# 0xMiden/miden-vm

Hardware: AMD Instinct MI355X
Metric: trace rows/sec proved (2^20-row trace, 96-bit sec) (higher is better)
Workload: dtype u64 (Goldilocks field, p = 2^64 - 2^32 + 1); 1 GPU; full proof of miden:20:51:8 (DummyMidenAir 2^20 x 51 + 8 EF aux), 96-bit production PCS params (blowup 8, FRI arity 4, 27 queries, PoW 4/12/16), Poseidon2 LMCS; trace resident in HBM, transcript on host; log_trace_rows=20, main_width=51, aux_width_ef=8, log_blowup=3, proof_bytes=137697, parallelism=1 GPU

## Files before the change

### miden-vm_amd/csrc/fri.hip

```cpp
#include <cstring>
#include "gl.cuh"
#include "../../include/midenhip.h"
#include "kernels.hpp"
#include "blake3.cuh"
#include "keccak.cuh"
#include "poseidon2_fast.cuh"
#define RESCUE_FAST 1
#include "rescue.cuh"
#include "salt.cuh"

__device__ __forceinline__ e2 ld_e2(const u64* p, size_t idx) {
  const ulonglong2 v = *reinterpret_cast<const ulonglong2*>(p + 2 * idx);
  return e2{v.x, v.y};
}
__device__ __forceinline__ void st_e2(u64* p, size_t idx, e2 v) { *reinterpret_cast<ulonglong2*>(p + 2 * idx) = make_ulonglong2(v.c0, v.c1); }

__device__ __forceinline__ u32 fri_row_pos(u32 p, int log_arity) { return bitrev32(p, log_arity); }

template <bool SALT>
__device__ __forceinline__ void fri_leaf_hash_body(const u64* __restrict__ ev, int log_rows , int cbits, int log_arity,
                                                   u64* __restrict__ digests, const SaltArgs* sa) {
  const int log_q = log_rows - log_arity;
  const size_t leaves = (size_t)1 << (log_q + cbits);
  const size_t s = blockIdx.x * (size_t)256 + threadIdx.x;
  if (s >= leaves) return;
  const size_t j = s >> log_q, r0 = s & (((size_t)1 << log_q) - 1);
  const u32 arity = 1u << log_arity;
  u64 st[12];
#pragma unroll
  for (int i = 0; i < 12; i++) st[i] = 0;
  for (u32 p0 = 0; p0 < arity; p0 += 4) {
#pragma unroll
    for (u32 k = 0; k < 4; k++) {
      e2 v = e2_make(0);
      if (p0 + k < arity) v = ld_e2(ev, (j << log_rows) + r0 + ((size_t)fri_row_pos(p0 + k, log_arity) << log_q));
      st[2 * k] = (p0 + k < arity) ? v.c0 : 0;
      st[2 * k + 1] = (p0 + k < arity) ? v.c1 : 0;
    }
    p2f_permute(st);
  }
  if constexpr (SALT) salt_absorb_p2(st, *sa, salt_phys_row(j, r0, cbits, log_q + cbits));
  ulonglong2* o = reinterpret_cast<ulonglong2*>(digests + 4 * s);
  o[0] = make_ulonglong2(st[0], st[1]);
  o[1] = make_ulonglong2(st[2], st[3]);
}
__global__ __launch_bounds__(256) void k_fri_leaf_hash(const u64* __restrict__ ev, int log_rows, int cbits, int log_arity,
                                                       u64* __restrict__ digests) {
  fri_leaf_hash_body<false>(ev, log_rows, cbits, log_arity, digests, nullptr);
}
__global__ __launch_bounds__(256) void k_fri_leaf_hash_salted(const u64* __restrict__ ev, int log_rows, int cbits, int log_arity,
                                                              u64* __restrict__ digests, SaltArgs sa) {
  fri_leaf_hash_body<true>(ev, log_rows, cbits, log_arity, digests, &sa);
}

template <bool SALT>
__device__ __forceinline__ void fri_leaf_hash_b3_body(const u64* __restrict__ ev, int log_rows, int cbits, int log_arity,
                                                      u64* __restrict__ digests, const SaltArgs* sa) {
  const int log_q = log_rows - log_arity;
  const size_t leaves = (size_t)1 << (log_q + cbits);
  const size_t s = blockIdx.x * (size_t)256 + threadIdx.x;
  if (s >= leaves) return;
  const size_t j = s >> log_q, r0 = s & (((size_t)1 << log_q) - 1);
  const u32 arity = 1u << log_arity;
  const u32 total = 32 + 16 * arity, n_blocks = (total + 63) / 64;
  b3::Stream h;
  h.init();
  uint32_t m[16], out[8];
#pragma unroll 1
  for (u32 b = 0; b < n_blocks; b++) {
    const int p0 = (int)(4 * b) - 2;
#pragma unroll
    for (int k = 0; k < 4; k++) {
      const int pp = p0 + k;
      e2 v = e2_make(0);
      if (pp >= 0 && (u32)pp < arity) v = ld_e2(ev, (j << log_rows) + r0 + ((size_t)fri_row_pos((u32)pp, log_arity) << log_q));
      m[4 * k] = (uint32_t)v.c0; m[4 * k + 1] = (uint32_t)(v.c0 >> 32);
      m[4 * k + 2] = (uint32_t)v.c1; m[4 * k + 3] = (uint32_t)(v.c1 >> 32);
    }
    if (b + 1 < n_blocks) h.block(m);
    else h.finish(m, total - 64 * b, out);
  }
  if constexpr (SALT) salt_absorb_b3(out, *sa, salt_phys_row(j, r0, cbits, log_q + cbits));
#pragma unroll
  for (int i = 0; i < 4; i++) digests[4 * s + i] = (u64)out[2 * i] | ((u64)out[2 * i + 1] << 32);
}
__global__ __launch_bounds__(256) void k_fri_leaf_hash_b3(const u64* __restrict__ ev, int log_rows, int cbits, int log_arity,
                                                          u64* __restrict__ digests) {
  fri_leaf_hash_b3_body<false>(ev, log_rows, cbits, log_arity, digests, nullptr);
}
__global__ __launch_bounds__(256) void k_fri_leaf_hash_b3_salted(const u64* __restrict__ ev, int log_rows, int cbits, int log_arity,
                                                                 u64* __restrict__ digests, SaltArgs sa) {
  fri_leaf_hash_b3_body<true>(ev, log_rows, cbits, log_arity, digests, &sa);
// ... 387 lines not shown
```

### miden-vm_amd/csrc/lmcs.hip

```cpp
#include "ctx.hpp"
#include "../../include/midenhip.h"
#include "kernels.hpp"
#include "poseidon2_fast.cuh"
#include "poseidon2_lanes.cuh"
#include "poseidon2_quad.cuh"
#include "blake3.cuh"
#include "keccak.cuh"
#define RESCUE_FAST 1
#include "rescue.cuh"
#include "gl.cuh"
#include "salt.cuh"
#include <algorithm>
#include <cstring>

static constexpr int LEAF_MAX_MATS = 8;
static constexpr int LEAF_THREADS = 256;

__global__ __launch_bounds__(256) void k_permute_soa(u64* st, size_t n) {
  size_t i = blockIdx.x * (size_t)blockDim.x + threadIdx.x;
  if (i >= n) return;
  u64 s[12];
#pragma unroll
  for (int j = 0; j < 12; j++) s[j] = st[j * n + i];
  p2f_permute(s);
// ... 20 lines not shown
double poseidon2_register_rate(mh_ctx* c) {
  const int blocks = 2048, iters = 64;
  DevBuf out((size_t)blocks * 256 * 8);
  hipEvent_t a = c->get_event(), b = c->get_event();
  MH_LAUNCH(k_perm_rate, dim3(blocks), dim3(256), 0, c->stream, out.u(), iters, 1ULL);
  double best = 0;
  for (int rep = 0; rep < 3; rep++) {
    HIP_CHECK(hipEventRecord(a, c->stream));
    MH_LAUNCH(k_perm_rate, dim3(blocks), dim3(256), 0, c->stream, out.u(), iters, 12345ULL + rep);
    HIP_CHECK(hipEventRecord(b, c->stream));
    HIP_CHECK(hipStreamSynchronize(c->stream));
    float ms = 0;
    HIP_CHECK(hipEventElapsedTime(&ms, a, b));
    best = std::max(best, (double)blocks * 256 * iters / (ms * 1e-3));
  }
  c->event_pool.push_back(a);
  c->event_pool.push_back(b);
  return best;
}

struct LeafMat {
  const u64* data;
  u32 width;
};
struct LeafArgs {
  LeafMat m[LEAF_MAX_MATS];
  int n_mats;
  int log_blowup;
  int log_n;
  const u64* state_in;
  int log_n_prev;
  u64* state_out;
  u64* digest_out;
  size_t q_begin, q_count;
};

template <bool SALT>
__device__ __forceinline__ void leaf_absorb_body(const LeafArgs& a, const SaltArgs* sa) {
  const size_t leaves = (size_t)1 << (a.log_n + a.log_blowup);
  const size_t q = a.q_begin + blockIdx.x * (size_t)blockDim.x + threadIdx.x;
  if (q >= (a.q_count ? a.q_begin + a.q_count : leaves)) return;
  const size_t j = q >> a.log_n, r = q & (((size_t)1 << a.log_n) - 1);
  u64 s[12];
  if (a.state_in) {
    const size_t leaves_prev = (size_t)1 << (a.log_n_prev + a.log_blowup);
    const size_t qi = (j << a.log_n_prev) + (r & (((size_t)1 << a.log_n_prev) - 1));
#pragma unroll
    for (int i = 0; i < 12; i++) s[i] = a.state_in[i * leaves_prev + qi];
  } else {
#pragma unroll
    for (int i = 0; i < 12; i++) s[i] = 0;
  }
  const size_t col_stride = leaves;
#pragma unroll 1
  for (int mi = 0; mi < a.n_mats; mi++) {
    const u64* base = a.m[mi].data + q;
    const u32 w = a.m[mi].width;
#pragma unroll 1
    for (u32 c0 = 0; c0 < w; c0 += 8) {
#pragma unroll
      for (int k = 0; k < 8; k++) s[k] = (c0 + k < w) ? base[(size_t)(c0 + k) * col_stride] : 0;
      p2f_permute(s);
    }
  }
  if constexpr (SALT) salt_absorb_p2(s, *sa, salt_phys_row(j, r, a.log_blowup, a.log_n + a.log_blowup));
  if (a.digest_out) {
    ulonglong2* o = reinterpret_cast<ulonglong2*>(a.digest_out + 4 * q);
    o[0] = make_ulonglong2(s[0], s[1]);
    o[1] = make_ulonglong2(s[2], s[3]);
  } else {
#pragma unroll
    for (int i = 0; i < 12; i++) a.state_out[i * leaves + q] = s[i];
  }
}
__global__ __launch_bounds__(LEAF_THREADS) void k_leaf_absorb(LeafArgs a) { leaf_absorb_body<false>(a, nullptr); }
__global__ __launch_bounds__(LEAF_THREADS) void k_leaf_absorb_salted(LeafArgs a, SaltArgs sa) { leaf_absorb_body<true>(a, &sa); }

template <bool SALT>
__device__ __forceinline__ void leaf_absorb_b3_body(const LeafArgs& a, const SaltArgs* sa) {
  const size_t leaves = (size_t)1 << (a.log_n + a.log_blowup);
  const size_t q = a.q_begin + blockIdx.x * (size_t)blockDim.x + threadIdx.x;
  if (q >= (a.q_count ? a.q_begin + a.q_count : leaves)) return;
  const size_t j = q >> a.log_n, r = q & (((size_t)1 << a.log_n) - 1);
  uint32_t st[8];
  if (a.state_in) {
    const size_t qi = (j << a.log_n_prev) + (r & (((size_t)1 << a.log_n_prev) - 1));
#pragma unroll
    for (int i = 0; i < 4; i++) {
      const u64 v = a.state_in[4 * qi + i];
      st[2 * i] = (uint32_t)v;
      st[2 * i + 1] = (uint32_t)(v >> 32);
    }
  } else {
#pragma unroll
    for (int i = 0; i < 8; i++) st[i] = 0;
  }
  const size_t col_stride = leaves;
#pragma unroll 1
  for (int mi = 0; mi < a.n_mats; mi++) {
    const u64* base = a.m[mi].data + q;
    const u32 w = a.m[mi].width;
    const u32 total = 32 + 8 * w;
    const u32 n_blocks = (total + 63) / 64;
    b3::Stream h;
    h.init();
    uint32_t m[16];
#pragma unroll 1
    for (u32 b = 0; b < n_blocks; b++) {
      const int f0 = (int)(8 * b) - 4;
#pragma unroll
      for (int k = 0; k < 8; k++) {
        const int f = f0 + k;
        u64 v = 0;
        if (f >= 0 && (u32)f < w) v = base[(size_t)f * col_stride];
        m[2 * k] = (uint32_t)v;
// ... 180 lines not shown
    if (e < sa.n) out[k * (size_t)sa.n + e] = z[e];
}
void lmcs_salt_rows(mh_ctx* c, const SaltArgs& salt, const u64* rows, size_t n_rows, u64* out) {
  if (!n_rows || !salt.n) return;
  MH_LAUNCH(k_salt_rows, dim3((unsigned)((n_rows + 255) / 256)), dim3(256), 0, c->stream, salt, rows, n_rows, out);
}
void lmcs_salt_assign(mh_ctx* c, mh_tree* t) {
  if (!c->salt.n) return;
  t->salt = c->salt;
  c->salt.tree++;
}
const SaltArgs* lmcs_salt_of(const mh_tree* t) { return t->salt.n ? &t->salt : nullptr; }
__global__ __launch_bounds__(256) void k_compress_kk(const u64* __restrict__ in, u64* __restrict__ out, size_t n_out, int log_n_coset) {
  const size_t q = blockIdx.x * (size_t)256 + threadIdx.x;
  if (q >= n_out) return;
  size_t l, rgt;
  if (log_n_coset >= 0) {
    const size_t N = (size_t)1 << log_n_coset;
    const size_t jp = q >> log_n_coset, r = q & (N - 1);
    l = ((2 * jp) << log_n_coset) + r;
    rgt = l + N;
  } else {
    l = 2 * q;
    rgt = l + 1;
  }
  uint64_t a[4], b[4], o[4];
#pragma unroll
  for (int i = 0; i < 4; i++) {
    a[i] = in[4 * l + i];
    b[i] = in[4 * rgt + i];
  }
  kk::compress_pair(a, b, o);
#pragma unroll
  for (int i = 0; i < 4; i++) out[4 * q + i] = o[i];
}

__global__ __launch_bounds__(256) void k_compress(const u64* __restrict__ in, u64* __restrict__ out, size_t n_out, int log_n_coset) {
  const size_t q = blockIdx.x * (size_t)blockDim.x + threadIdx.x;
  if (q >= n_out) return;
  size_t l, rgt;
  if (log_n_coset >= 0) {
    size_t N = (size_t)1 << log_n_coset;
    size_t jp = q >> log_n_coset, r = q & (N - 1);
    l = ((2 * jp) << log_n_coset) + r;
    rgt = l + N;
  } else {
    l = 2 * q;
    rgt = l + 1;
  }
  const ulonglong2* pl = reinterpret_cast<const ulonglong2*>(in + 4 * l);
  const ulonglong2* pr = reinterpret_cast<const ulonglong2*>(in + 4 * rgt);
  ulonglong2 l0 = pl[0], l1 = pl[1], r0 = pr[0], r1 = pr[1];
  u64 s[12] = {l0.x, l0.y, l1.x, l1.y, r0.x, r0.y, r1.x, r1.y, 0, 0, 0, 0};
  p2f_permute(s);
  ulonglong2* o = reinterpret_cast<ulonglong2*>(out + 4 * q);
  o[0] = make_ulonglong2(s[0], s[1]);
  o[1] = make_ulonglong2(s[2], s[3]);
}

static size_t compress_lanes_max_nodes() {
  static const size_t v = [] {
    const char* e = getenv("MH_LANES_MAX_NODES");
    return e ? (size_t)atol(e) : (size_t)8192;
  }();
  return v;
}
__global__ __launch_bounds__(256) void k_compress_lanes(const u64* __restrict__ in, u64* __restrict__ out, size_t n_out, int log_n_coset) {
  const size_t node = (blockIdx.x * (size_t)256 + threadIdx.x) >> 4;
  const int g = threadIdx.x & 15;
  const bool active = node < n_out;
  const size_t q = active ? node : 0;
  size_t l, rgt;
  if (log_n_coset >= 0) {
    const size_t N = (size_t)1 << log_n_coset;
    const size_t jp = q >> log_n_coset, r = q & (N - 1);
    l = ((2 * jp) << log_n_coset) + r;
    rgt = l + N;
  } else {
    l = 2 * q;
    rgt = l + 1;
  }
  const u64* src = in + 4 * (g < 4 ? l : rgt) + (g & 3);
  u64 s = g < 8 ? *src : 0;
  s = p2l_permute(s);
  if (active && g < 4) out[4 * q + g] = s;
}

static size_t compress_quad_min_nodes() {
  static const size_t v = [] {
    const char* e = getenv("MH_QUAD_MIN_NODES");
    return e ? (size_t)atol(e) : (size_t)16384;
  }();
  return v;
}
static size_t compress_quad_max_nodes() {
  static const size_t v = [] {
    const char* e = getenv("MH_QUAD_MAX_NODES");
    return e ? (size_t)atol(e) : (size_t)32768;
  }();
  return v;
}
__global__ __launch_bounds__(256) void k_compress_quad(const u64* __restrict__ in, u64* __restrict__ out, size_t n_out, int log_n_coset) {
  const size_t node = (blockIdx.x * (size_t)256 + threadIdx.x) >> 2;
  const int j = threadIdx.x & 3;
  const bool active = node < n_out;
  const size_t q = active ? node : 0;
  size_t l, rgt;
// ... 388 lines not shown
```

### miden-vm_amd/csrc/p2_fast_constants.inc

```
static const unsigned long long P2F_ARK_INT_SCALED[22] = {
  0x4adf842aa75d4316ULL, 0xc7ddc3945255a751ULL, 0x3a16dbc6b75abaa6ULL, 0x4160d6694e06fff1ULL,
  0xe022996682de326cULL, 0xc8e9d874293bba12ULL, 0xa2e2b15ade3b7d8fULL, 0x9b6dac180ec943cfULL,
  0xe8bb7136f94d695dULL, 0xf12458f8ebe4789bULL, 0x1dc193fff01be2b6ULL, 0xb68e807d90fed489ULL,
  0x1e4085d70c946015ULL, 0x66a5e58521b4c3c6ULL, 0x53b280ba8b2f8249ULL, 0xe4d602af8c2cf37eULL,
  0x813ee2a294c44327ULL, 0x813b943e27068773ULL, 0x9abe7bd4fb69436eULL, 0x12f583e142599766ULL,
  0x3798883e37881f6bULL, 0xed264b0c16fc039fULL,
};
static const unsigned long long P2F_INT_K[22] = {
  0x0000000000000001ULL, 0xffffbfff00004001ULL, 0xefffffff00000001ULL, 0xfffffbff00000001ULL,
  0xfffffffeff000001ULL, 0xfffffffeffffffc1ULL, 0x000ffffffff00000ULL, 0x00000003fffffffcULL,
  0x0001000000000000ULL, 0x0000000040000000ULL, 0x0000000000001000ULL, 0xfbffffff04000001ULL,
  0xfffffeff00000101ULL, 0xffbfffff00000001ULL, 0xffffffef00000001ULL, 0xfffffffefffc0001ULL,
  0xffffffff00000000ULL, 0x00003fffffffc000ULL, 0x1000000000000000ULL, 0x0000040000000000ULL,
  0x0000000001000000ULL, 0x0000000000000040ULL,
};
static const unsigned long long P2F_DESCALE = 0xfffffffec0000001ULL;
static const unsigned long long P2G_ARK[22] = {
  0x4adf842aa75d4316ULL, 0x8fbb8729a4ab4ea1ULL, 0x742db78d6eb5754cULL, 0x82c1acd29c0dffe2ULL,
  0xc04532ce05bc64d7ULL, 0x91d3b0e952777423ULL, 0x45c562b6bc76fb1dULL, 0x36db58311d92879dULL,
  0xd176e26ef29ad2b9ULL, 0xe248b1f2d7c8f135ULL, 0x3b8327ffe037c56cULL, 0x6d1d00fc21fda911ULL,
  0x3c810bae1928c02aULL, 0xcd4bcb0a4369878cULL, 0xa7650175165f0492ULL, 0xc9ac05601859e6fbULL,
  0x027dc5462988864dULL, 0x0277287d4e0d0ee5ULL, 0x357cf7aaf6d286dbULL, 0x25eb07c284b32eccULL,
  0x6f31107c6f103ed6ULL, 0xda4c96192df8073dULL,
};
static const unsigned long long P2G_K[22] = {
  0x0000000000000002ULL, 0xfffffeff00000101ULL, 0xffbfffff00000001ULL, 0xffffffef00000001ULL,
  0xfffffffefffc0001ULL, 0xffffffff00000000ULL, 0x00003fffffffc000ULL, 0x1000000000000000ULL,
  0x0000040000000000ULL, 0x0000000001000000ULL, 0x0000000000000040ULL, 0xffefffff00100001ULL,
  0xfffffffb00000005ULL, 0xfffeffff00000001ULL, 0xfffffffec0000001ULL, 0xfffffffefffff001ULL,
  0x03fffffffc000000ULL, 0x000000ffffffff00ULL, 0x0040000000000000ULL, 0x0000001000000000ULL,
  0x0000000000040000ULL, 0x0000000000000001ULL,
};
static const unsigned long long P2G_DESCALE = 0xfffffffee0000001ULL;
static constexpr int P2F_INT_K_LOG2[22] = {0, 174, 156, 138, 120, 102, 84, 66, 48, 30, 12, 186, 168, 150, 132, 114, 96, 78, 60, 42, 24, 6};
static constexpr int P2F_DESCALE_LOG2 = 126;
static constexpr int P2G_K_LOG2[22] = {1, 168, 150, 132, 114, 96, 78, 60, 42, 24, 6, 180, 162, 144, 126, 108, 90, 72, 54, 36, 18, 0};
static constexpr int P2G_DESCALE_LOG2 = 125;
```

### miden-vm_amd/csrc/poseidon2_fast.cuh

```cuda
#pragma once
#include "poseidon2.cuh"

namespace p2c {
#include "p2_fast_constants.inc"
}

#ifndef P2F_ASM
#define P2F_ASM 1
#endif
#ifndef P2F_GROUP
#define P2F_GROUP 4
#endif

#if defined(__HIP_DEVICE_COMPILE__)

template <u32 K>
__device__ __forceinline__ u64 p2f_mad(u64 acc, u32 x) {
  u64 d, cy;
  asm("v_mad_u64_u32 %0, %1, %2, %3, %4" : "=v"(d), "=s"(cy) : "v"(x), "n"(K), "v"(acc));
  return d;
}
template <u32 K>
__device__ __forceinline__ u64 p2f_zmul(u32 x) {
  u64 d, cy;
  asm("v_mad_u64_u32 %0, %1, %2, %3, 0" : "=v"(d), "=s"(cy) : "v"(x), "n"(K));
  return d;
}
__device__ __forceinline__ u32 lo32(u64 x) { return (u32)x; }
__device__ __forceinline__ u32 hi32(u64 x) { return (u32)(x >> 32); }

__device__ __forceinline__ u64 p2f_mul_c(u64 a, u64 b) {
  const u32 a0 = lo32(a), a1 = hi32(a), b0 = lo32(b), b1 = hi32(b);
  const u64 p00 = (u64)a0 * b0;
  const u64 m = (u64)a0 * b1 + (p00 >> 32);
  const u64 m2 = (u64)a1 * b0 + (u32)m;
  const u64 hi = (u64)a1 * b1 + (m >> 32) + (m2 >> 32);
  const u64 lo = (m2 << 32) | (u32)p00;
  const u32 x2 = lo32(hi), x3 = hi32(hi);
  u64 t = (u64)x2 * 0xFFFFFFFFu + lo;
  t += (t < lo) ? GL_EPS : 0;
  u64 r = t - x3;
  r -= (t < x3) ? GL_EPS : 0;
  return r;
}
#define P2F_A asm volatile
#ifndef P2F_GAP_NOPS
#define P2F_GAP_NOPS 1
#endif
#define P2F_GAP()                                          \
  do {                                                     \
    if (P2F_GAP_NOPS && N == 1) P2F_A("s_nop 1");          \
    else if (P2F_GAP_NOPS && N == 2) P2F_A("s_nop 0");     \
  } while (0)
#define P2F_SCR(i, PRE, POST, ...)                                                  \
  do {                                                                              \
    switch ((i) & 7) {                                                              \
      case 0: P2F_A(PRE "s[84:85]" POST : __VA_ARGS__ : "s84", "s85"); break;        \
      case 1: P2F_A(PRE "s[86:87]" POST : __VA_ARGS__ : "s86", "s87"); break;        \
      case 2: P2F_A(PRE "s[88:89]" POST : __VA_ARGS__ : "s88", "s89"); break;        \
      case 3: P2F_A(PRE "s[90:91]" POST : __VA_ARGS__ : "s90", "s91"); break;        \
      case 4: P2F_A(PRE "s[92:93]" POST : __VA_ARGS__ : "s92", "s93"); break;        \
      case 5: P2F_A(PRE "s[94:95]" POST : __VA_ARGS__ : "s94", "s95"); break;        \
      case 6: P2F_A(PRE "s[96:97]" POST : __VA_ARGS__ : "s96", "s97"); break;        \
      default: P2F_A(PRE "s[98:99]" POST : __VA_ARGS__ : "s98", "s99"); break;       \
    }                                                                               \
  } while (0)
#define P2F_MAD0(i, D, X, Y) P2F_SCR(i, "v_mad_u64_u32 %0, ", ", %1, %2, 0", "=v"(D) : "v"(X), "v"(Y))
#define P2F_MADA(i, D, X, Y, ACC) P2F_SCR(i, "v_mad_u64_u32 %0, ", ", %1, %2, %3", "=v"(D) : "v"(X), "v"(Y), "v"(ACC))
#define P2F_CARRY_IN(i, OP, D, X, C) P2F_SCR(i, OP " %0, ", ", %1, 0, %2", "=v"(D) : "v"(X), "s"(C))
#define P2F_MAD0S(i, D, X, Y) P2F_SCR(i, "v_mad_u64_u32 %0, ", ", %1, %2, 0", "=v"(D) : "v"(X), "s"(Y))
#define P2F_MADAS(i, D, X, Y, ACC) P2F_SCR(i, "v_mad_u64_u32 %0, ", ", %1, %2, %3", "=v"(D) : "v"(X), "s"(Y), "v"(ACC))
template <int N, bool BS = false>
__device__ __forceinline__ void p2f_mulN(u64 (&r)[N], const u64 (&a)[N], const u64 (&b)[N]) {
  u64 p00[N], m[N], hi[N], t[N];
  u64 cm[N], k1[N], k2[N], k3[N], c1[N], bb[N], bw[N], c3[N];
  u32 w1[N], accl[N], acch[N], rl[N], rh[N];
#pragma unroll
  for (int i = 0; i < N; i++) {
    if constexpr (BS) P2F_MAD0S(i, p00[i], lo32(a[i]), lo32(b[i]));
    else P2F_MAD0(i, p00[i], lo32(a[i]), lo32(b[i]));
  }
#pragma unroll
  for (int i = 0; i < N; i++) {
    if constexpr (BS) P2F_MAD0S(i, m[i], lo32(a[i]), hi32(b[i]));
    else P2F_MAD0(i, m[i], lo32(a[i]), hi32(b[i]));
  }
#pragma unroll
  for (int i = 0; i < N; i++) {
    if constexpr (BS) P2F_A("v_mad_u64_u32 %0, %1, %2, %3, %4" : "=v"(m[i]), "=s"(cm[i]) : "v"(hi32(a[i])), "s"(lo32(b[i])), "0"(m[i]));
    else P2F_A("v_mad_u64_u32 %0, %1, %2, %3, %4" : "=v"(m[i]), "=s"(cm[i]) : "v"(hi32(a[i])), "v"(lo32(b[i])), "0"(m[i]));
  }
#pragma unroll
  for (int i = 0; i < N; i++) P2F_A("v_add_co_u32_e64 %0, %1, %2, %3" : "=v"(w1[i]), "=s"(k1[i]) : "v"(hi32(p00[i])), "v"(lo32(m[i])));
  P2F_GAP();
#pragma unroll
  for (int i = 0; i < N; i++) P2F_A("v_addc_co_u32_e64 %0, %1, %2, 0, %3" : "=v"(accl[i]), "=s"(k2[i]) : "v"(hi32(m[i])), "s"(k1[i]));
#pragma unroll
  for (int i = 0; i < N; i++)
    k3[i] = cm[i] | k2[i];
#pragma unroll
  for (int i = 0; i < N; i++) {
    const u32 zero = 0;
    P2F_CARRY_IN(i, "v_addc_co_u32_e64", acch[i], zero, k3[i]);
  }
#pragma unroll
  for (int i = 0; i < N; i++) {
    const u64 acc = ((u64)acch[i] << 32) | accl[i];
    if constexpr (BS) P2F_MADAS(i, hi[i], hi32(a[i]), hi32(b[i]), acc);
    else P2F_MADA(i, hi[i], hi32(a[i]), hi32(b[i]), acc);
  }
#pragma unroll
  for (int i = 0; i < N; i++) {
    const u64 lo = ((u64)w1[i] << 32) | lo32(p00[i]);
    P2F_A("v_mad_u64_u32 %0, %1, %2, -1, %3" : "=v"(t[i]), "=s"(c1[i]) : "v"(lo32(hi[i])), "v"(lo));
  }
  P2F_GAP();
#pragma unroll
  for (int i = 0; i < N; i++) P2F_A("v_subb_co_u32_e64 %0, %1, %2, %3, %4" : "=v"(rl[i]), "=s"(bb[i]) : "v"(lo32(t[i])), "v"(hi32(hi[i])), "s"(c1[i]));
#pragma unroll
  for (int i = 0; i < N; i++) P2F_CARRY_IN(i, "v_addc_co_u32_e64", rh[i], hi32(t[i]), c1[i]);
  if (P2F_GAP_NOPS && N == 1) P2F_A("s_nop 0");
#pragma unroll
  for (int i = 0; i < N; i++) P2F_A("v_subb_co_u32_e64 %0, %1, %2, 0, %3" : "=v"(rh[i]), "=s"(bw[i]) : "0"(rh[i]), "s"(bb[i]));
  P2F_GAP();
#pragma unroll
  for (int i = 0; i < N; i++) P2F_A("v_addc_co_u32_e64 %0, %1, %2, 0, %3" : "=v"(rl[i]), "=s"(c3[i]) : "0"(rl[i]), "s"(bw[i]));
#pragma unroll
  for (int i = 0; i < N; i++) k3[i] = bw[i] & ~c3[i];
#pragma unroll
  for (int i = 0; i < N; i++) {
    P2F_CARRY_IN(i, "v_subb_co_u32_e64", rh[i], rh[i], k3[i]);
    r[i] = ((u64)rh[i] << 32) | rl[i];
  }
}
#undef P2F_GAP
#undef P2F_SCR
#undef P2F_MAD0
#undef P2F_MADA
#undef P2F_MAD0S
#undef P2F_MADAS
#undef P2F_CARRY_IN
__device__ __forceinline__ u64 p2f_mul_nv(u64 a, u64 b) {
  u64 p00, m, hi, t, d0, d1, d2, d3, d4, d5, cm, k1, k2, c1, bb, bw, c3;
  u32 w1, accl, acch, rl, rh;
  const u32 zero = 0;
  asm("v_mad_u64_u32 %0, %1, %2, %3, 0" : "=v"(p00), "=s"(d0) : "v"(lo32(a)), "v"(lo32(b)));
  asm("v_mad_u64_u32 %0, %1, %2, %3, 0" : "=v"(m), "=s"(d1) : "v"(lo32(a)), "v"(hi32(b)));
  asm("v_mad_u64_u32 %0, %1, %2, %3, %4" : "=v"(m), "=s"(cm) : "v"(hi32(a)), "v"(lo32(b)), "0"(m));
  asm("v_add_co_u32_e64 %0, %1, %2, %3" : "=v"(w1), "=s"(k1) : "v"(hi32(p00)), "v"(lo32(m)));
  asm("s_nop 1\n\tv_addc_co_u32_e64 %0, %1, %2, 0, %3" : "=v"(accl), "=s"(k2) : "v"(hi32(m)), "s"(k1));
  const u64 k3 = cm | k2;
  asm("v_addc_co_u32_e64 %0, %1, %2, 0, %3" : "=v"(acch), "=s"(d2) : "v"(zero), "s"(k3));
  const u64 acc = ((u64)acch << 32) | accl;
  asm("v_mad_u64_u32 %0, %1, %2, %3, %4" : "=v"(hi), "=s"(d3) : "v"(hi32(a)), "v"(hi32(b)), "v"(acc));
  const u64 lo = ((u64)w1 << 32) | lo32(p00);
  asm("v_mad_u64_u32 %0, %1, %2, -1, %3" : "=v"(t), "=s"(c1) : "v"(lo32(hi)), "v"(lo));
  asm("s_nop 1\n\tv_subb_co_u32_e64 %0, %1, %2, %3, %4" : "=v"(rl), "=s"(bb) : "v"(lo32(t)), "v"(hi32(hi)), "s"(c1));
  asm("s_nop 1\n\tv_addc_co_u32_e64 %0, %1, %2, 0, %3" : "=v"(rh), "=s"(d4) : "v"(hi32(t)), "s"(c1));
  asm("s_nop 1\n\tv_subb_co_u32_e64 %0, %1, %2, 0, %3" : "=v"(rh), "=s"(bw) : "0"(rh), "s"(bb));
  asm("s_nop 1\n\tv_addc_co_u32_e64 %0, %1, %2, 0, %3" : "=v"(rl), "=s"(c3) : "0"(rl), "s"(bw));
  const u64 mk = bw & ~c3;
  asm("v_subb_co_u32_e64 %0, %1, %2, 0, %3" : "=v"(rh), "=s"(d5) : "0"(rh), "s"(mk));
  return ((u64)rh << 32) | rl;
}
__device__ __forceinline__ u64 p2f_mul(u64 a, u64 b) {
#if P2F_ASM
  u64 r[1];
  const u64 x[1] = {a}, y[1] = {b};
  p2f_mulN<1>(r, x, y);
  return r[0];
#else
  return p2f_mul_c(a, b);
#endif
}
__device__ __forceinline__ u64 p2f_mul_k(u64 a, u64 k) {
#if P2F_ASM
  u64 r[1];
  const u64 x[1] = {a}, y[1] = {k};
  p2f_mulN<1, true>(r, x, y);
  return r[0];
#else
  return p2f_mul_c(a, k);
#endif
}
__device__ __forceinline__ u64 p2f_sbox(u64 x) {
#if P2F_ASM
  const u64 x2 = p2f_mul(x, x);
  u64 q[2];
  const u64 qa[2] = {x2, x2}, qb[2] = {x, x2};
  p2f_mulN<2>(q, qa, qb);
  return p2f_mul(q[0], q[1]);
#else
  const u64 x2 = p2f_mul(x, x);
  const u64 x3 = p2f_mul(x2, x);
  const u64 x4 = p2f_mul(x2, x2);
  return p2f_mul(x3, x4);
#endif
}
__device__ __forceinline__ void p2f_sbox12(u64 s[12]) {
#if P2F_ASM
#pragma unroll
  for (int g = 0; g < 12; g += P2F_GROUP) {
    u64 x[P2F_GROUP], x2[P2F_GROUP], x3[P2F_GROUP];
#pragma unroll
    for (int i = 0; i < P2F_GROUP; i++) x[i] = s[g + i];
    p2f_mulN<P2F_GROUP>(x2, x, x);
    p2f_mulN<P2F_GROUP>(x3, x2, x);
    p2f_mulN<P2F_GROUP>(x, x2, x2);
    p2f_mulN<P2F_GROUP>(x2, x3, x);
#pragma unroll
    for (int i = 0; i < P2F_GROUP; i++) s[g + i] = x2[i];
  }
#else
#pragma unroll
  for (int i = 0; i < 12; i++) s[i] = p2f_sbox(s[i]);
#endif
}
__device__ __forceinline__ u64 p2f_add_canon(u64 x, u64 c) {
  u64 s = x + c;
  s += (s < c) ? GL_EPS : 0;
  return s;
}
__device__ __forceinline__ u64 p2f_fold(u64 L, u64 H) {
  const u64 m = (u64)hi32(H) * 0xFFFFFFFFu + L;
  const u32 hl = lo32(H);
  const u32 s = hi32(m) + hl;
  u64 r = ((u64)s << 32) | lo32(m);
  r += (s < hl) ? GL_EPS : 0;
  return r;
}
__device__ __forceinline__ u64 p2f_fold_signed(u64 L, u64 H) {
  const u64 BL = ((u64)1 << 30) + ((u64)1 << 62);
  const u64 BH = ((u64)1 << 30) * 0xFFFFFFFFULL - ((u64)1 << 30);
  return p2f_fold(L + BL, H + BH);
}

__host__ __device__ constexpr int p2f_shl_sign(int E, int part, int w) {
  constexpr int tab[3][2][3] = {{{1, 0, -1}, {0, 1, 1}}, {{0, -1, -1}, {1, 1, 0}}, {{-1, -1, 0}, {1, 0, -1}}};
  const int e = E % 96, sg = tab[e / 32][part][w] * (E >= 96 ? -1 : 1);
  return (w == 2 && e % 32 == 0) ? 0 : sg;
}
template <int E>
__device__ __forceinline__ void p2f_shl_words(u64 y, u32 (&u)[3]) {
  static_assert(E >= 0 && E < 192, "exponent out of range");
  constexpr int b = E % 96 % 32;
  const u64 z = y << b;
  u[0] = lo32(z);
  u[1] = hi32(z);
  if constexpr (b > 0) u[2] = hi32(y) >> (32 - b);
  else u[2] = 0;
}
template <int SG>
__device__ __forceinline__ u64 p2f_acc_word(u64 acc, u32 u) {
  if constexpr (SG > 0) return p2f_mad<1>(acc, u);
  else if constexpr (SG < 0) return acc - (u64)u;
  else return acc;
}
template <int E, int PART, int SG>
__device__ __forceinline__ u64 p2f_acc_shl(u64 acc, const u32 (&u)[3]) {
  acc = p2f_acc_word<SG * p2f_shl_sign(E, PART, 0)>(acc, u[0]);
  acc = p2f_acc_word<SG * p2f_shl_sign(E, PART, 1)>(acc, u[1]);
  return p2f_acc_word<SG * p2f_shl_sign(E, PART, 2)>(acc, u[2]);
}
#define P2F_IC(F, r) F(std::integral_constant<int, r>{})
#define P2F_ROUNDS22(F)                                                                                               \
  do {                                                                                                                \
    P2F_IC(F, 0); P2F_IC(F, 1); P2F_IC(F, 2); P2F_IC(F, 3); P2F_IC(F, 4); P2F_IC(F, 5); P2F_IC(F, 6); P2F_IC(F, 7);          \
    P2F_IC(F, 8); P2F_IC(F, 9); P2F_IC(F, 10); P2F_IC(F, 11); P2F_IC(F, 12); P2F_IC(F, 13); P2F_IC(F, 14); P2F_IC(F, 15);    \
    P2F_IC(F, 16); P2F_IC(F, 17); P2F_IC(F, 18); P2F_IC(F, 19); P2F_IC(F, 20); P2F_IC(F, 21);                             \
  } while (0)
template <int E, int PART>
__device__ __forceinline__ void p2f_pm_shl(u64 R, const u32 (&u)[3], u64& s8, u64& n) {
  constexpr int plus = (p2f_shl_sign(E, PART, 0) > 0) + (p2f_shl_sign(E, PART, 1) > 0) + (p2f_shl_sign(E, PART, 2) > 0);
  constexpr int minus = (p2f_shl_sign(E, PART, 0) < 0) + (p2f_shl_sign(E, PART, 1) < 0) + (p2f_shl_sign(E, PART, 2) < 0);
  if constexpr (plus >= minus) {
    s8 = p2f_acc_shl<E, PART, 1>(R, u) << 3;
    n = (R << 4) - s8;
  } else {
    n = p2f_acc_shl<E, PART, -1>(R, u) << 3;
    s8 = (R << 4) - n;
  }
}

template <bool RC>
__device__ __forceinline__ void p2f_external(u64 s[12], const unsigned long long* rc) {
  u64 oL[12], oH[12];
#pragma unroll
  for (int i = 0; i < 12; i += 4) {
#pragma unroll
    for (int part = 0; part < 2; part++) {
      const u32 a = part ? hi32(s[i]) : lo32(s[i]), b = part ? hi32(s[i + 1]) : lo32(s[i + 1]);
      const u32 c = part ? hi32(s[i + 2]) : lo32(s[i + 2]), d = part ? hi32(s[i + 3]) : lo32(s[i + 3]);
      const u64 t01 = p2f_mad<1>(p2f_zmul<1>(a), b);
      const u64 t23 = p2f_mad<1>(p2f_zmul<1>(c), d);
      const u64 t0123 = t01 + t23;
      const u64 t01123 = p2f_mad<1>(t0123, b);
      const u64 t01233 = p2f_mad<1>(t0123, d);
      u64* o = part ? oH : oL;
      o[i + 3] = p2f_mad<2>(t01233, a);
      o[i + 1] = p2f_mad<2>(t01123, c);
      o[i] = t01123 + t01;
      o[i + 2] = t01233 + t23;
    }
  }
#pragma unroll
  for (int l = 0; l < 4; l++) {
    const u64 stL = oL[l] + oL[4 + l] + oL[8 + l], stH = oH[l] + oH[4 + l] + oH[8 + l];
#pragma unroll
    for (int i = l; i < 12; i += 4) {
      u64 L = oL[i] + stL, H = oH[i] + stH;
      if (RC) {
        L += rc[i] & 0xFFFFFFFFULL;
        H += rc[i] >> 32;
      }
      s[i] = p2f_fold(L, H);
    }
  }
}

__device__ __forceinline__ void p2f_permute(u64 s[12]) {
  p2f_external<true>(s, p2c::P2_ARK_EXT_INITIAL);
#pragma unroll 1
  for (int r = 0; r < 4; r++) {
    p2f_sbox12(s);
    if (r < 3) {
      p2f_external<true>(s, p2c::P2_ARK_EXT_INITIAL + 12 * (r + 1));
    } else {
      p2f_external<false>(s, nullptr);
    }
  }
  u64 t0 = p2f_add_canon(s[0], p2c::P2G_ARK[0]);
  u64 X1L, X1H, X2L, X2H, X11L, X11H;
  u64 AL[4], AH[4], BL[4], BH[4];
  {
    u32 y[3];
    p2f_shl_words<p2c::P2G_K_LOG2[0]>(p2f_sbox(t0), y);
    u64 RL = p2f_zmul<1>(lo32(s[1])), RH = p2f_zmul<1>(hi32(s[1]));
#pragma unroll
    for (int i = 2; i < 12; i++) {
      RL = p2f_mad<1>(RL, lo32(s[i]));
      RH = p2f_mad<1>(RH, hi32(s[i]));
    }
    u64 s8L, s8H, nL, nH;
    p2f_pm_shl<p2c::P2G_K_LOG2[0], 0>(RL << 1, y, s8L, nL);
    p2f_pm_shl<p2c::P2G_K_LOG2[0], 1>(RH << 1, y, s8H, nH);
    {
      const u64 rc = p2c::P2G_ARK[1];
      t0 = p2f_fold_signed(nL + (rc & 0xFFFFFFFFULL), nH + (rc >> 32));
    }
    X1L = p2f_mad<16>(s8L, lo32(s[1])), X1H = p2f_mad<16>(s8H, hi32(s[1]));
    X2L = p2f_mad<32>(s8L, lo32(s[2])), X2H = p2f_mad<32>(s8H, hi32(s[2]));
    X11L = p2f_mad<2>(s8L, lo32(s[11])), X11H = p2f_mad<2>(s8H, hi32(s[11]));
#define P2G_PAIR0(q, i, j, K)                                                         \
  AL[q] = p2f_mad<1>(p2f_zmul<1>(lo32(s[i])), lo32(s[j]));                            \
  AH[q] = p2f_mad<1>(p2f_zmul<1>(hi32(s[i])), hi32(s[j]));                            \
  BL[q] = p2f_mad<K>(s8L, lo32(s[i])) - p2f_zmul<K>(lo32(s[j]));                      \
  BH[q] = p2f_mad<K>(s8H, hi32(s[i])) - p2f_zmul<K>(hi32(s[j]));
    P2G_PAIR0(0, 3, 6, 4)
    P2G_PAIR0(1, 4, 7, 24)
    P2G_PAIR0(2, 5, 8, 32)
    P2G_PAIR0(3, 9, 10, 2)
#undef P2G_PAIR0
  }
#define P2G_ROUND(r, CL, CH, PL, PH, HAS_RC)                                                             \
  {                                                                                                       \
    u32 y[3];                            \
    p2f_shl_words<p2c::P2G_K_LOG2[r]>(p2f_sbox(t0), y);                                                   \
    const u64 RL = ((CL[0] + CL[1] + CL[2] + CL[3]) << 1) + X1L + X2L + X11L;                             \
    const u64 RH = ((CH[0] + CH[1] + CH[2] + CH[3]) << 1) + X1H + X2H + X11H;                             \
    u64 s8L, s8H, nL, nH;                                 \
    p2f_pm_shl<p2c::P2G_K_LOG2[r], 0>(RL, y, s8L, nL);                                                    \
    p2f_pm_shl<p2c::P2G_K_LOG2[r], 1>(RH, y, s8H, nH);                                                    \
    {                                                                                                     \
      if (HAS_RC) {                                                                                       \
        const u64 rc = p2c::P2G_ARK[(r) + 1];                                                             \
        nL += rc & 0xFFFFFFFFULL;                                                                         \
        nH += rc >> 32;                                                                                   \
      }                                                                                                   \
      t0 = p2f_fold_signed(nL, nH);                                                                       \
    }                                                                                                     \
    X1L = (X1L << 3) + s8L, X1H = (X1H << 3) + s8H;                                                       \
    X2L = (X2L << 4) + s8L, X2H = (X2H << 4) + s8H;                                                       \
    X11L += s8L, X11H += s8H;                                                                             \
    PL[0] = (PL[0] << 4) + s8L, PH[0] = (PH[0] << 4) + s8H;                                      \
// ... 11 lines not shown
    const u64 v = p2f_fold_signed(L_, H_);        \
    L_ = p2f_zmul<1>(lo32(v));                    \
    H_ = p2f_zmul<1>(hi32(v));                    \
  }
  const auto round_pair = [&](auto rr) {
    constexpr int r = decltype(rr)::value;
    P2G_ROUND(r, BL, BH, AL, AH, r < 21)
    if constexpr ((r & 3) == 3) {
      P2G_REFOLD(X1L, X1H)
      P2G_REFOLD(X2L, X2H)
      P2G_REFOLD(X11L, X11H)
#pragma unroll
      for (int q = 0; q < 4; q++) {
        P2G_REFOLD(AL[q], AH[q])
        P2G_REFOLD(BL[q], BH[q])
      }
    }
    if constexpr (r + 1 < 22) P2G_ROUND(r + 1, AL, AH, BL, BH, true)
  };
  round_pair(std::integral_constant<int, 1>{});
  round_pair(std::integral_constant<int, 3>{});
  round_pair(std::integral_constant<int, 5>{});
  round_pair(std::integral_constant<int, 7>{});
  round_pair(std::integral_constant<int, 9>{});
  round_pair(std::integral_constant<int, 11>{});
  round_pair(std::integral_constant<int, 13>{});
  round_pair(std::integral_constant<int, 15>{});
  round_pair(std::integral_constant<int, 17>{});
  round_pair(std::integral_constant<int, 19>{});
  round_pair(std::integral_constant<int, 21>{});
#undef P2G_ROUND
#undef P2G_REFOLD
  s[0] = t0;
  s[1] = p2f_fold_signed(X1L, X1H);
  s[2] = p2f_fold_signed(X2L, X2H);
  s[11] = p2f_fold_signed(X11L, X11H);
#define P2G_UNPAIR(q, i, j, KL, KH)                         \
  {                                                         \
    const u64 kL = KL, kH = KH;                             \
    s[i] = p2f_fold_signed(AL[q] + kL, AH[q] + kH);         \
    s[j] = p2f_fold_signed(AL[q] - kL, AH[q] - kH);         \
  }
  P2G_UNPAIR(0, 3, 6, BL[0] << 2, BH[0] << 2)
  P2G_UNPAIR(1, 4, 7, ((BL[1] << 1) + BL[1]) << 3, ((BH[1] << 1) + BH[1]) << 3)
  P2G_UNPAIR(2, 5, 8, BL[2] << 5, BH[2] << 5)
  P2G_UNPAIR(3, 9, 10, BL[3] << 1, BH[3] << 1)
#undef P2G_UNPAIR
#if P2F_ASM
#pragma unroll
  for (int g = 0; g < 12; g += 4) {
    u64 x[4], k[4];
#pragma unroll
    for (int i = 0; i < 4; i++) { x[i] = s[g + i]; k[i] = p2c::P2G_DESCALE; }
    p2f_mulN<4>(x, x, k);
#pragma unroll
    for (int i = 0; i < 4; i++) s[g + i] = x[i];
  }
#else
#pragma unroll
  for (int i = 0; i < 12; i++) s[i] = p2f_mul(s[i], p2c::P2G_DESCALE);
#endif
#pragma unroll
  for (int i = 0; i < 12; i++) s[i] = p2f_add_canon(s[i], p2c::P2_ARK_EXT_TERMINAL[i]);
#pragma unroll 1
  for (int r = 0; r < 4; r++) {
    p2f_sbox12(s);
    if (r < 3) {
      p2f_external<true>(s, p2c::P2_ARK_EXT_TERMINAL + 12 * (r + 1));
    } else {
      p2f_external<false>(s, nullptr);
    }
  }
#pragma unroll
  for (int i = 0; i < 12; i++) s[i] = gl_canon(s[i]);
}

#else
__device__ void p2f_permute(u64 s[12]);
__device__ u64 p2f_mul(u64 a, u64 b);
__device__ u64 p2f_mul_nv(u64 a, u64 b);
__device__ u64 p2f_mul_k(u64 a, u64 k);
__device__ u64 p2f_sbox(u64 x);
__device__ void p2f_sbox12(u64 s[12]);
__device__ u32 lo32(u64 x);
__device__ u32 hi32(u64 x);
#endif
```

Baseline: 24.35 million trace rows/s.

## Fold Poseidon2 round constants into multiply addends and trim final-round outputs

Round constants are folded into the v_mad_u64_u32 addend of the last s-box multiply, using precomputed constant tables, instead of separate add-with-reduce passes. The permutation is split into a body and a tail, and the tail's last external linear layer computes only the outputs a caller needs: capacity lanes for intermediate sponge absorbs, digest lanes for final hashes. The aim is fewer ALU ops per Poseidon2 permutation in leaf hashing, FRI leaf hashing and Merkle compression. It adds a correctness dependency on the new constant tables and on the correct partial-output selection.

Result: faster. 24.80 million trace rows/s (median of 6 runs) (+1.8%).

```diff
diff --git a/miden-vm_amd/csrc/fri.hip b/miden-vm_amd/csrc/fri.hip
--- a/miden-vm_amd/csrc/fri.hip
+++ b/miden-vm_amd/csrc/fri.hip
@@ -37,7 +37,10 @@
       st[2 * k] = (p0 + k < arity) ? v.c0 : 0;
       st[2 * k + 1] = (p0 + k < arity) ? v.c1 : 0;
     }
-    p2f_permute(st);
+    p2f_body(st);
+    if (p0 + 4 < arity) p2f_tail<P2F_CAPACITY>(st);
+    else if (SALT) p2f_tail<P2F_ALL>(st);
+    else p2f_tail<P2F_DIGEST>(st);
   }
   if constexpr (SALT) salt_absorb_p2(st, *sa, salt_phys_row(j, r0, cbits, log_q + cbits));
   ulonglong2* o = reinterpret_cast<ulonglong2*>(digests + 4 * s);
diff --git a/miden-vm_amd/csrc/lmcs.hip b/miden-vm_amd/csrc/lmcs.hip
--- a/miden-vm_amd/csrc/lmcs.hip
+++ b/miden-vm_amd/csrc/lmcs.hip
@@ -96,6 +96,10 @@
     for (int i = 0; i < 12; i++) s[i] = 0;
   }
   const size_t col_stride = leaves;
+  int last_mi = -1;
+#pragma unroll 1
+  for (int mi = 0; mi < a.n_mats; mi++)
+    if (a.m[mi].width) last_mi = mi;
 #pragma unroll 1
   for (int mi = 0; mi < a.n_mats; mi++) {
     const u64* base = a.m[mi].data + q;
@@ -104,7 +108,10 @@
     for (u32 c0 = 0; c0 < w; c0 += 8) {
 #pragma unroll
       for (int k = 0; k < 8; k++) s[k] = (c0 + k < w) ? base[(size_t)(c0 + k) * col_stride] : 0;
-      p2f_permute(s);
+      p2f_body(s);
+      if (!(mi == last_mi && c0 + 8 >= w)) p2f_tail<P2F_CAPACITY>(s);
+      else if (SALT || !a.digest_out) p2f_tail<P2F_ALL>(s);
+      else p2f_tail<P2F_DIGEST>(s);
     }
   }
   if constexpr (SALT) salt_absorb_p2(s, *sa, salt_phys_row(j, r, a.log_blowup, a.log_n + a.log_blowup));
@@ -391,7 +398,8 @@
   const ulonglong2* pr = reinterpret_cast<const ulonglong2*>(in + 4 * rgt);
   ulonglong2 l0 = pl[0], l1 = pl[1], r0 = pr[0], r1 = pr[1];
   u64 s[12] = {l0.x, l0.y, l1.x, l1.y, r0.x, r0.y, r1.x, r1.y, 0, 0, 0, 0};
-  p2f_permute(s);
+  p2f_body(s);
+  p2f_tail<P2F_DIGEST>(s);
   ulonglong2* o = reinterpret_cast<ulonglong2*>(out + 4 * q);
   o[0] = make_ulonglong2(s[0], s[1]);
   o[1] = make_ulonglong2(s[2], s[3]);
diff --git a/miden-vm_amd/csrc/p2_fast_constants.inc b/miden-vm_amd/csrc/p2_fast_constants.inc
--- a/miden-vm_amd/csrc/p2_fast_constants.inc
+++ b/miden-vm_amd/csrc/p2_fast_constants.inc
@@ -36,3 +36,61 @@
 static constexpr int P2F_DESCALE_LOG2 = 126;
 static constexpr int P2G_K_LOG2[22] = {1, 168, 150, 132, 114, 96, 78, 60, 42, 24, 6, 180, 162, 144, 126, 108, 90, 72, 54, 36, 18, 0};
 static constexpr int P2G_DESCALE_LOG2 = 125;
+alignas(64) static const unsigned long long P2F_EXT_K[192] = {
+  0x00000000a6be4018ULL, 0x0000000006704035ULL, 0x00000000410d0225ULL, 0x00000000acb8e7f1ULL,
+  0x00000000706db6a1ULL, 0x00000000e9a34ef7ULL, 0x00000000cdd7998dULL, 0x00000000a675f2d0ULL,
+  0x000000004c6071f3ULL, 0x000000006da4e37bULL, 0x000000004b0a3657ULL, 0x000000004a8307c2ULL,
+  0x00000000b9de6343ULL, 0x0000000097ff40ddULL, 0x0000000065c3a3ecULL, 0x00000000d561847aULL,
+  0x00000000c76ab334ULL, 0x00000000513262c0ULL, 0x000000001e44c0cdULL, 0x000000008e20a3a0ULL,
+  0x00000000f83e7de7ULL, 0x0000000051b9d6f3ULL, 0x000000003fae1f22ULL, 0x000000006c169fe7ULL,
+  0x000000006a4d2ebeULL, 0x000000004552daaaULL, 0x000000003d7c83bfULL, 0x000000004661cca5ULL,
+  0x000000009796f8b2ULL, 0x000000002bfb38f3ULL, 0x00000000f0630852ULL, 0x0000000009dbf49aULL,
+  0x00000000fccf17e4ULL, 0x000000000f97ac14ULL, 0x00000000923a8fadULL, 0x00000000b3d1497dULL,
+  0x0000000084282a03ULL, 0x00000000b36f8bf0ULL, 0x00000000d7fa867cULL, 0x000000006ec45e8dULL,
+  0x00000000aea9463cULL, 0x00000000c0aa7027ULL, 0x0000000049757723ULL, 0x00000000a89c18c6ULL,
+  0x00000000d05127c2ULL, 0x000000002e82d2a9ULL, 0x000000006099c852ULL, 0x00000000009bb588ULL,
+  0x00000000b65e92a6ULL, 0x00000000e143eadaULL, 0x000000000e847554ULL, 0x000000006f3420a9ULL,
+  0x000000007b21ed38ULL, 0x00000000ac14fc8eULL, 0x000000009d338c07ULL, 0x00000000b4840326ULL,
+  0x0000000028f145e5ULL, 0x00000000d4a52d9dULL, 0x000000001336fe91ULL, 0x000000009df4bb00ULL,
+  0x000000000996cff4ULL, 0x0000000087d13248ULL, 0x000000007038e736ULL, 0x000000003bbd0959ULL,
+  0x0000000051b19be8ULL, 0x00000000421108a7ULL, 0x000000000be438fcULL, 0x0000000089fa37ccULL,
+  0x000000001947d887ULL, 0x00000000a52048b7ULL, 0x00000000a196d505ULL, 0x000000009edd306bULL,
+  0x000000006dff5206ULL, 0x000000008bde367fULL, 0x00000000ec82e369ULL, 0x000000002d8f985fULL,
+  0x00000000ee7e218fULL, 0x0000000000a315dfULL, 0x00000000ed80827cULL, 0x000000001719571fULL,
+  0x0000000030aae4a9ULL, 0x0000000026b5edd5ULL, 0x00000000b129b433ULL, 0x000000009b7acd34ULL,
+  0x0000000005d5f4d1ULL, 0x00000000aa744e0aULL, 0x000000005b7fd482ULL, 0x00000000a2f78d9fULL,
+  0x0000000030aae4a9ULL, 0x0000000026b5edd5ULL, 0x00000000b129b433ULL, 0x000000009b7acd34ULL,
+  0x0000000005d5f4d1ULL, 0x00000000aa744e0aULL, 0x000000005b7fd482ULL, 0x00000000a2f78d9fULL,
+  0x0000000062ebfdaaULL, 0x000000007c3cf91aULL, 0x0000000061abfc5aULL, 0x000000007b086fa3ULL,
+  0x00000000205d0e0fULL, 0x00000000991c073aULL, 0x000000006464be3dULL, 0x00000000e0054092ULL,
+  0x0000000090654560ULL, 0x00000000d1e0d1a6ULL, 0x0000000036da84e8ULL, 0x000000006a07999cULL,
+  0x00000000efab1c24ULL, 0x0000000039d95334ULL, 0x00000000b6acd66cULL, 0x000000007cecfd2eULL,
+  0x0000000031dd52b4ULL, 0x00000000989aa7cdULL, 0x0000000022353a44ULL, 0x00000000eedc5e3dULL,
+  0x0000000036b29e5eULL, 0x00000000e70c12fdULL, 0x00000000679383a3ULL, 0x00000000346ab037ULL,
+  0x00000000f777c90aULL, 0x0000000038ca4098ULL, 0x0000000065dc98e6ULL, 0x000000008b47a811ULL,
+  0x0000000005a78bfdULL, 0x00000000cc345c9aULL, 0x00000000697a126cULL, 0x0000000031bc7757ULL,
+  0x000000005a10b42dULL, 0x00000000d86e4de5ULL, 0x00000000d069fe37ULL, 0x000000004af5ed8cULL,
+  0x00000000c8c17f8cULL, 0x00000000cf5fd7ecULL, 0x00000000b64ae544ULL, 0x00000000a9d2b6f8ULL,
+  0x00000000a24ca08aULL, 0x000000006cfd1803ULL, 0x000000006e697c21ULL, 0x0000000041fee543ULL,
+  0x00000000705ac331ULL, 0x000000005dd29d2dULL, 0x000000001f8145f1ULL, 0x00000000fcf55f92ULL,
+  0x000000003465b56fULL, 0x0000000014a42d71ULL, 0x00000000e2fbf3edULL, 0x00000000645ba451ULL,
+  0x00000000b0357649ULL, 0x00000000b7fad45dULL, 0x00000000e759726bULL, 0x0000000007172fe7ULL,
+  0x00000000940b9b93ULL, 0x0000000034365772ULL, 0x000000007e27f13fULL, 0x00000000dd9ebf4cULL,
+  0x00000000c21454d9ULL, 0x0000000021f6818cULL, 0x00000000e9b1eaadULL, 0x00000000bd3003d0ULL,
+  0x000000001ad14bd2ULL, 0x000000003db4f1e8ULL, 0x0000000087e84aacULL, 0x00000000fc6e8921ULL,
+  0x00000000fba9105cULL, 0x00000000f5b67f47ULL, 0x000000009caffcc8ULL, 0x00000000b0271febULL,
+  0x0000000000000000ULL, 0x0000000000000000ULL, 0x0000000000000000ULL, 0x0000000000000000ULL,
+  0x0000000000000000ULL, 0x0000000000000000ULL, 0x0000000000000000ULL, 0x0000000000000000ULL,
+  0x0000000000000000ULL, 0x0000000000000000ULL, 0x0000000000000000ULL, 0x0000000000000000ULL,
+  0x0000000000000000ULL, 0x0000000000000000ULL, 0x0000000000000000ULL, 0x0000000000000000ULL,
+  0x0000000000000000ULL, 0x0000000000000000ULL, 0x0000000000000000ULL, 0x0000000000000000ULL,
+  0x0000000000000000ULL, 0x0000000000000000ULL, 0x0000000000000000ULL, 0x0000000000000000ULL,
+};
+static const unsigned long long P2F_TERM0_K[24] = {
+  0x000000004882a24dULL, 0x00000000c68be7c9ULL, 0x000000005cdaedd9ULL, 0x00000000af996d5dULL,
+  0x00000000e7daf6a5ULL, 0x000000009717f025ULL, 0x000000006e7216f4ULL, 0x000000006436679eULL,
+  0x00000000047af267ULL, 0x000000008a223d99ULL, 0x00000000a133ba9aULL, 0x00000000bb512e35ULL,
+  0x000000007671aa03ULL, 0x00000000fbbf4409ULL, 0x00000000f6811e61ULL, 0x00000000f04058ebULL,
+  0x000000003fac7ffbULL, 0x000000005cca8470ULL, 0x000000005de6469fULL, 0x000000009b55c794ULL,
+  0x00000000808e934fULL, 0x000000008e05bf09ULL, 0x00000000876307d7ULL, 0x000000002ea900deULL,
+};
diff --git a/miden-vm_amd/csrc/poseidon2_fast.cuh b/miden-vm_amd/csrc/poseidon2_fast.cuh
--- a/miden-vm_amd/csrc/poseidon2_fast.cuh
+++ b/miden-vm_amd/csrc/poseidon2_fast.cuh
@@ -10,6 +10,16 @@
 #endif
 #ifndef P2F_GROUP
 #define P2F_GROUP 4
+#endif
+#ifndef P2F_RC_ADDEND
+#define P2F_RC_ADDEND 1
+#endif
+#if !P2F_ASM
+#undef P2F_RC_ADDEND
+#define P2F_RC_ADDEND 0
+#endif
+#ifndef P2F_TAILS
+#define P2F_TAILS 1
 #endif
 
 #if defined(__HIP_DEVICE_COMPILE__)
@@ -70,19 +80,23 @@
 #define P2F_CARRY_IN(i, OP, D, X, C) P2F_SCR(i, OP " %0, ", ", %1, 0, %2", "=v"(D) : "v"(X), "s"(C))
 #define P2F_MAD0S(i, D, X, Y) P2F_SCR(i, "v_mad_u64_u32 %0, ", ", %1, %2, 0", "=v"(D) : "v"(X), "s"(Y))
 #define P2F_MADAS(i, D, X, Y, ACC) P2F_SCR(i, "v_mad_u64_u32 %0, ", ", %1, %2, %3", "=v"(D) : "v"(X), "s"(Y), "v"(ACC))
-template <int N, bool BS = false>
-__device__ __forceinline__ void p2f_mulN(u64 (&r)[N], const u64 (&a)[N], const u64 (&b)[N]) {
+#define P2F_MADK(i, D, X, Y, K) P2F_SCR(i, "v_mad_u64_u32 %0, ", ", %1, %2, %3", "=v"(D) : "v"(X), "v"(Y), "s"(K))
+template <int N, bool BS = false, bool KA = false>
+__device__ __forceinline__ void p2f_mulN(u64 (&r)[N], const u64 (&a)[N], const u64 (&b)[N], const unsigned long long* ka = nullptr) {
+  static_assert(!(BS && KA), "one scalar operand per VOP3 instruction: b in SGPRs and an SGPR addend exclude each other");
   u64 p00[N], m[N], hi[N], t[N];
   u64 cm[N], k1[N], k2[N], k3[N], c1[N], bb[N], bw[N], c3[N];
   u32 w1[N], accl[N], acch[N], rl[N], rh[N];
 #pragma unroll
   for (int i = 0; i < N; i++) {
     if constexpr (BS) P2F_MAD0S(i, p00[i], lo32(a[i]), lo32(b[i]));
+    else if constexpr (KA) P2F_MADK(i, p00[i], lo32(a[i]), lo32(b[i]), ka[2 * i]);
     else P2F_MAD0(i, p00[i], lo32(a[i]), lo32(b[i]));
   }
 #pragma unroll
   for (int i = 0; i < N; i++) {
     if constexpr (BS) P2F_MAD0S(i, m[i], lo32(a[i]), hi32(b[i]));
+    else if constexpr (KA) P2F_MADK(i, m[i], lo32(a[i]), hi32(b[i]), ka[2 * i + 1]);
     else P2F_MAD0(i, m[i], lo32(a[i]), hi32(b[i]));
   }
 #pragma unroll
@@ -139,6 +153,7 @@
 #undef P2F_MADA
 #undef P2F_MAD0S
 #undef P2F_MADAS
+#undef P2F_MADK
 #undef P2F_CARRY_IN
 __device__ __forceinline__ u64 p2f_mul_nv(u64 a, u64 b) {
   u64 p00, m, hi, t, d0, d1, d2, d3, d4, d5, cm, k1, k2, c1, bb, bw, c3;
@@ -197,7 +212,20 @@
   return p2f_mul(x3, x4);
 #endif
 }
-__device__ __forceinline__ void p2f_sbox12(u64 s[12]) {
+template <int W>
+__device__ __forceinline__ void p2f_load_k(unsigned long long (&d)[W], const unsigned long long* k) {
+  if constexpr (W == 8) {
+    typedef unsigned long long k8 __attribute__((ext_vector_type(8)));
+    const k8 v = *reinterpret_cast<const k8*>(k);
+#pragma unroll
+    for (int i = 0; i < 8; i++) d[i] = v[i];
+  } else {
+#pragma unroll
+    for (int i = 0; i < W; i++) d[i] = k[i];
+  }
+}
+template <bool KA = false>
+__device__ __forceinline__ void p2f_sbox12(u64 s[12], const unsigned long long* k = nullptr) {
 #if P2F_ASM
 #pragma unroll
   for (int g = 0; g < 12; g += P2F_GROUP) {
@@ -207,11 +235,18 @@
     p2f_mulN<P2F_GROUP>(x2, x, x);
     p2f_mulN<P2F_GROUP>(x3, x2, x);
     p2f_mulN<P2F_GROUP>(x, x2, x2);
-    p2f_mulN<P2F_GROUP>(x2, x3, x);
+    if constexpr (KA) {
+      unsigned long long kg[2 * P2F_GROUP];
+      p2f_load_k(kg, k + 2 * g);
+      p2f_mulN<P2F_GROUP, false, true>(x2, x3, x, kg);
+    } else {
+      p2f_mulN<P2F_GROUP>(x2, x3, x);
+    }
 #pragma unroll
     for (int i = 0; i < P2F_GROUP; i++) s[g + i] = x2[i];
   }
 #else
+  static_assert(!KA, "addends need the asm form of the product");
 #pragma unroll
   for (int i = 0; i < 12; i++) s[i] = p2f_sbox(s[i]);
 #endif
@@ -282,7 +317,11 @@
   }
 }
 
-template <bool RC>
+enum { P2F_ALL = 0, P2F_DIGEST = 1, P2F_CAPACITY = 2 };
+__host__ __device__ constexpr bool p2f_out_has(int out, int i) {
+  return out == P2F_ALL || (out == P2F_DIGEST && i < 4) || (out == P2F_CAPACITY && i >= 8);
+}
+template <bool RC, int OUT = P2F_ALL>
 __device__ __forceinline__ void p2f_external(u64 s[12], const unsigned long long* rc) {
   u64 oL[12], oH[12];
 #pragma unroll
@@ -308,6 +347,7 @@
     const u64 stL = oL[l] + oL[4 + l] + oL[8 + l], stH = oH[l] + oH[4 + l] + oH[8 + l];
 #pragma unroll
     for (int i = l; i < 12; i += 4) {
+      if (!p2f_out_has(OUT, i)) continue;
       u64 L = oL[i] + stL, H = oH[i] + stH;
       if (RC) {
         L += rc[i] & 0xFFFFFFFFULL;
@@ -318,8 +358,15 @@
   }
 }
 
-__device__ __forceinline__ void p2f_permute(u64 s[12]) {
+__device__ __forceinline__ void p2f_body(u64 s[12]) {
   p2f_external<true>(s, p2c::P2_ARK_EXT_INITIAL);
+#if P2F_RC_ADDEND
+#pragma unroll 1
+  for (int r = 0; r < 4; r++) {
+    p2f_sbox12<true>(s, p2c::P2F_EXT_K + 24 * r);
+    p2f_external<false>(s, nullptr);
+  }
+#else
 #pragma unroll 1
   for (int r = 0; r < 4; r++) {
     p2f_sbox12(s);
@@ -329,7 +376,12 @@
       p2f_external<false>(s, nullptr);
     }
   }
+#endif
+#if P2F_RC_ADDEND
+  u64 t0 = s[0];
+#else
   u64 t0 = p2f_add_canon(s[0], p2c::P2G_ARK[0]);
+#endif
   u64 X1L, X1H, X2L, X2H, X11L, X11H;
   u64 AL[4], AH[4], BL[4], BH[4];
   {
@@ -447,7 +499,11 @@
     u64 x[4], k[4];
 #pragma unroll
     for (int i = 0; i < 4; i++) { x[i] = s[g + i]; k[i] = p2c::P2G_DESCALE; }
+#if P2F_RC_ADDEND
+    p2f_mulN<4, false, true>(x, x, k, p2c::P2F_TERM0_K + 2 * g);
+#else
     p2f_mulN<4>(x, x, k);
+#endif
 #pragma unroll
     for (int i = 0; i < 4; i++) s[g + i] = x[i];
   }
@@ -455,23 +511,44 @@
 #pragma unroll
   for (int i = 0; i < 12; i++) s[i] = p2f_mul(s[i], p2c::P2G_DESCALE);
 #endif
+#if !P2F_RC_ADDEND
 #pragma unroll
   for (int i = 0; i < 12; i++) s[i] = p2f_add_canon(s[i], p2c::P2_ARK_EXT_TERMINAL[i]);
+#endif
 #pragma unroll 1
-  for (int r = 0; r < 4; r++) {
+  for (int r = 0;; r++) {
+#if P2F_RC_ADDEND
+    p2f_sbox12<true>(s, p2c::P2F_EXT_K + 24 * (4 + r));
+    if (r == 3) break;
+    p2f_external<false>(s, nullptr);
+#else
     p2f_sbox12(s);
-    if (r < 3) {
-      p2f_external<true>(s, p2c::P2_ARK_EXT_TERMINAL + 12 * (r + 1));
-    } else {
-      p2f_external<false>(s, nullptr);
-    }
-  }
-#pragma unroll
-  for (int i = 0; i < 12; i++) s[i] = gl_canon(s[i]);
-}
-
-#else
+    if (r == 3) break;
+    p2f_external<true>(s, p2c::P2_ARK_EXT_TERMINAL + 12 * (r + 1));
+#endif
+  }
+}
+template <int OUT>
+__device__ __forceinline__ void p2f_tail(u64 s[12]) {
+  constexpr int O = P2F_TAILS ? OUT : (int)P2F_ALL;
+  p2f_external<false, O>(s, nullptr);
+  if constexpr (O != P2F_CAPACITY) {
+#pragma unroll
+    for (int i = 0; i < 12; i++)
+      if (p2f_out_has(O, i)) s[i] = gl_canon(s[i]);
+  }
+}
+__device__ __forceinline__ void p2f_permute(u64 s[12]) {
+  p2f_body(s);
+  p2f_tail<P2F_ALL>(s);
+}
+
+#else
+enum { P2F_ALL = 0, P2F_DIGEST = 1, P2F_CAPACITY = 2 };
 __device__ void p2f_permute(u64 s[12]);
+__device__ void p2f_body(u64 s[12]);
+template <int OUT>
+__device__ void p2f_tail(u64 s[12]);
 __device__ u64 p2f_mul(u64 a, u64 b);
 __device__ u64 p2f_mul_nv(u64 a, u64 b);
 __device__ u64 p2f_mul_k(u64 a, u64 k);
```
